# JialeTao/MRFA

Hardware: AMD Instinct MI355X
Metric: frames/sec (256x256 source+driving pair) fwd+bwd (higher is better)
Workload: dtype f32; 1 GPU; vox1.yaml MTIA (TokenPose_B) prior + DenseMotion + RaftFlow refinement, 256x256, bs=8/GPU, fwd+bwd+clip+Adam, train-mode BN, surrogate L1 loss; global_batch=8, parallelism=dp1, prior=mtia, background_predictor=False, sync_bn=False, launch=hipGraph, optimizer=FlatAdam (K20), mfma=bf16x6

## Files before the change

### mrfa_amd/csrc/common.h

```cpp
#pragma once
#include <hip/hip_runtime.h>
#include <stdio.h>
#include <string.h>
#include "mrfa_hip.h"

typedef float f32x16 __attribute__((ext_vector_type(16)));
typedef float f32x4 __attribute__((ext_vector_type(4)));

void mrfa_set_error(const char* fmt, ...);

struct MrfaTuning {
    int conv_small;
    int conv_halo, conv_halo_min_tiles, conv_halo_pr, conv_halo_phase, conv_halo_bn256, conv_halo_bn192, conv_halo_bn64_fill;
    int conv_lean, conv_lean_min_wgs, conv_lean_geo, gemm_lean;
    int wgrad_halo, wgrad_halo_min_wgs, wgrad_halo_target_wgs, wgrad_halo_phase, wgrad_lean;
    int conv_fewout3, attention_mfma;
};
extern MrfaTuning g_tune;

struct HaloGeo { int PR, BN; bool phase; };

enum class ConvFamily { lean, gemm_lean, small, halo, halo_dgrad, rows_split, rows_f32, refused };
struct ConvPlan {
    ConvFamily family;
    char error[256];
    long long M;
    int KT;
    int lean_geo, gemm_cfg, small_tm, small_tn;
    HaloGeo halo;
    int BM, BN, splitk;
    bool w8;
    bool fused;
    bool fin_in_launch;
    bool reads_w;
    int last_config;
    bool groups_ok, bst_ok, stride2_ok, mask_ok, phase_dgrad_ok;
};
ConvPlan plan_conv(const mrfa_conv_params& p);

enum class WgradFamily { lean, small, halo, tiled, refused };
struct WgradPlan {
    WgradFamily family;
    char error[192];
    long long M;
    bool lean, small;
    bool groups_ok, stride2_ok;
};
WgradPlan plan_wgrad(const mrfa_wgrad_params& p);

int mrfa_conv_split_launch(hipStream_t st, const mrfa_conv_params& p, int KT, long long M, int splitk, int BN);
bool mrfa_conv_halo_eligible(const mrfa_conv_params& p, HaloGeo* geo);
int mrfa_conv_halo_launch(hipStream_t st, const mrfa_conv_params& p, const HaloGeo& geo);
int mrfa_wgrad_split_launch(hipStream_t st, const mrfa_wgrad_params& p, dim3 grid, long long M, long long kps, int tiles_n, int nsplit, int inner,
                            int total_splits, int taps, long long partial_stride, int BM, int BN);

bool mrfa_wgrad_halo_eligible(const mrfa_wgrad_params& p);
int mrfa_wgrad_halo_launch(hipStream_t st, const mrfa_wgrad_params& p);

bool mrfa_fewout3_wgrad(hipStream_t st, const float* x, int ldx, int N, int H, int W, int Cin, const float* dy, int lddy, int Cout, int R, int pad,
                        float* dw, float* dbias, int* rc);

int mrfa_conv_lean_pick(const mrfa_conv_params& p);
int mrfa_conv_lean_launch(hipStream_t st, const mrfa_conv_params& p, int geo);
int mrfa_gemm_lean_pick(const mrfa_conv_params& p, long long M);
int mrfa_gemm_lean_launch(hipStream_t st, const mrfa_conv_params& p, long long M, int cfg);

bool mrfa_conv_small_eligible(const mrfa_conv_params& p, long long M);
int mrfa_conv_small_launch(hipStream_t st, const mrfa_conv_params& p, long long M, int tm, int tn);

bool mrfa_attention_mfma_ok(int d, int n, const void* qkv, int ld, const void* out, int ldo, const void* dout, int lddo, const void* dqkv, int lddq);
int mrfa_attention_fwd_mfma(hipStream_t st, const float* qkv, int ld, int B, int n, int heads, int d, float scale, float* out, int ldo, float* lse);
int mrfa_attention_bwd_mfma(hipStream_t st, const float* qkv, int ld, const float* out, int ldo, const float* dout, int lddo, const float* lse,
                            float* delta, int B, int n, int heads, int d, float scale, float* dqkv, int lddq);

bool mrfa_wgrad_lean_eligible(const mrfa_wgrad_params& p);
int mrfa_wgrad_lean_multi(hipStream_t st, const mrfa_wgrad_params* ps, int n, unsigned char* taken);

bool mrfa_wgrad_small_eligible(const mrfa_wgrad_params& p, long long M);
int mrfa_wgrad_small_launch(hipStream_t st, const mrfa_wgrad_params& p, long long M);

#define MRFA_CHECK_ARG(cond, ...)                      \
    do {                                               \
        if (!(cond)) {                                 \
            mrfa_set_error(__VA_ARGS__);               \
            return 1;                                  \
        }                                              \
    } while (0)

#define MRFA_CHECK_LAUNCH(name)                                                   \
    do {                                                                          \
        hipError_t e_ = hipGetLastError();                                        \
        if (e_ != hipSuccess) {                                                   \
            mrfa_set_error("%s: launch failed: %s", name, hipGetErrorString(e_)); \
            return 2;                                                             \
        }                                                                         \
    } while (0)

static inline bool aligned16(const void* p) { return (reinterpret_cast<uintptr_t>(p) & 15u) == 0; }
static inline int cdiv(long long a, long long b) { return (int)((a + b - 1) / b); }
// ... 107 lines not shown
```

### mrfa_amd/csrc/conv_plan.hip

```cpp
#include "common.h"
#include <stdarg.h>

MrfaTuning g_tune = {
     1,
     1,  128,  0,  1,  1,
     1,  1,
     1,  128,  -1,
     1,
     1,  192,  256,  1,
     1,
     1,  1,
};

enum TuneKind { T_ON, T_INT, T_NONNEG, T_NONNEG_ON, T_LEVEL, T_POS };
static const struct { const char* key; int* field; TuneKind kind; } TUNING_KEYS[] = {
    {"conv_small", &g_tune.conv_small, T_ON},
    {"conv_halo", &g_tune.conv_halo, T_ON},
    {"conv_halo_min_tiles", &g_tune.conv_halo_min_tiles, T_INT},
    {"conv_halo_pr", &g_tune.conv_halo_pr, T_INT},
    {"conv_halo_phase", &g_tune.conv_halo_phase, T_ON},
    {"conv_halo_bn256", &g_tune.conv_halo_bn256, T_ON},
    {"conv_halo_bn192", &g_tune.conv_halo_bn192, T_ON},
    {"conv_halo_bn64_fill", &g_tune.conv_halo_bn64_fill, T_ON},
    {"conv_lean", &g_tune.conv_lean, T_ON},
    {"conv_lean_min_wgs", &g_tune.conv_lean_min_wgs, T_NONNEG},
    {"conv_lean_geo", &g_tune.conv_lean_geo, T_INT},
    {"gemm_lean", &g_tune.gemm_lean, T_LEVEL},
    {"wgrad_halo", &g_tune.wgrad_halo, T_ON},
    {"wgrad_halo_min_wgs", &g_tune.wgrad_halo_min_wgs, T_NONNEG},
    {"wgrad_halo_target_wgs", &g_tune.wgrad_halo_target_wgs, T_POS},
    {"wgrad_halo_phase", &g_tune.wgrad_halo_phase, T_NONNEG_ON},
    {"wgrad_lean", &g_tune.wgrad_lean, T_ON},
    {"conv_fewout3", &g_tune.conv_fewout3, T_ON},
    {"attention_mfma", &g_tune.attention_mfma, T_ON},
};

extern "C" int mrfa_set_tuning(const char* key, int value) {
    if (!key) return -1;
    for (const auto& k : TUNING_KEYS) {
        if (strcmp(key, k.key)) continue;
        const int prev = *k.field;
        switch (k.kind) {
            case T_ON: *k.field = value != 0; break;
            case T_INT: *k.field = value; break;
            case T_NONNEG: if (value >= 0) *k.field = value; break;
            case T_NONNEG_ON: if (value >= 0) *k.field = value != 0; break;
            case T_LEVEL: if (value >= 0) *k.field = value > 2 ? 2 : value; break;
            case T_POS: if (value > 0) *k.field = value; break;
        }
        return prev;
    }
    return -1;
}

namespace {
constexpr int BK = 32;

template <typename Plan>
Plan& refuse(Plan& c, const char* fmt, ...) {
    va_list ap;
    va_start(ap, fmt);
    vsnprintf(c.error, sizeof(c.error), fmt, ap);
    va_end(ap);
    c.family = decltype(c.family)::refused;
    return c;
}

void plan_rows(ConvPlan& c, const mrfa_conv_params& p, int mode) {
    const bool flat = p.kflat > 0;
    const long long M = c.M;
    const int KT = c.KT;
    const int nb = p.nbatch > 1 ? p.nbatch : 1;
    int BN = 128;
    {
        const int cands[4] = {128, 96, 64, 32};
        const double pen[4] = {1.0, 1.08, 1.16, 1.3};
        double best = 1e18;
        for (int i = 0; i < 4; ++i) {
            if (cands[i] == 96 && flat) continue;
            const double cost = (double)cdiv(p.Cout, cands[i]) * cands[i] * pen[i];
            if (cost < best) { best = cost; BN = cands[i]; }
        }
    }
    if (mode >= 1 && !flat && p.Cout >= 32) BN = p.Cout <= 64 ? 64 : 128;
    auto ntiles = [&](int bm, int bn) { return ((M + bm - 1) / bm) * cdiv(p.Cout, bn) * nb; };
    int BM = 128;
    if (BN == 96 && ntiles(128, 96) < 384) BN = 128;
    if (BN == 128) { if (M <= 32) BM = 32; else if (M <= 64) BM = 64; }
    else if (BN == 64 && M <= 64) BM = 64;
    int splitk = 1;
    const bool auto_split = (p.splitk == 0);
    if (p.splitk > 1) splitk = p.splitk;
    {
        const bool short_k_big_m = KT < 32 && M > 4096;
        const bool grouped_stats = p.groups > 1 && p.stats && !(p.sk_ticket && !p.accumulate);
        const int max_split = (auto_split && !short_k_big_m && !grouped_stats) ? (KT / 2 > 0 ? KT / 2 : 1) : 1;
        long long t = ntiles(BM, BN);
        if (t < 384 && !(short_k_big_m && t >= 128)) {
            const bool half_target = auto_split && p.sk_ticket && !p.accumulate && KT >= 72 && KT <= 320 && BM == 128 && t >= 8 && t <= 16;
            int want = (int)(((half_target ? 256 : 512) + t - 1) / t);
            if (auto_split) splitk = want <= max_split ? want : max_split;
            const int min_bm = (BN == 128) ? 32 : (BN == 64 ? 64 : 128);
            while (!half_target && ntiles(BM, BN) * splitk < 384 && BM > min_bm) {
                BM >>= 1;
                if (auto_split) {
                    t = ntiles(BM, BN);
                    want = (int)((512 + t - 1) / t);
                    splitk = want <= max_split ? want : max_split;
                }
            }
            if (splitk < 1) splitk = 1;
        }
    }
    bool w8 = false;
    if (p.tile) {
        BM = p.tile >> 16; BN = p.tile & 0x7fff; w8 = (p.tile & 0x8000) != 0;
        if (p.splitk >= 1) splitk = p.splitk;
// ... 134 lines not shown
```

### mrfa_amd/csrc/sample.hip

```cpp
#include "mfma_bf16.h"

namespace {

struct Taps {
    int x0, y0;
    float fx, fy;
};

__device__ __forceinline__ Taps make_taps(float ix, float iy) {
    Taps t;
    const float fx0 = floorf(ix), fy0 = floorf(iy);
    t.x0 = (int)fx0;
    t.y0 = (int)fy0;
    t.fx = ix - fx0;
    t.fy = iy - fy0;
    return t;
}


struct Taps4 {
    size_t o00, o01, o10, o11;
    float w00, w01, w10, w11;
    float fx, fy;
    bool ok00, ok01, ok10, ok11;
// ... 107 lines not shown
        const u32x4 r10 = *reinterpret_cast<const u32x4*>(base + tp.o10 * ldi), r11 = *reinterpret_cast<const u32x4*>(base + tp.o11 * ldi);
        f32x4 a00, b00, a01, b01, a10, b10, a11, b11;
        widen8(r00, a00, b00); widen8(r01, a01, b01); widen8(r10, a10, b10); widen8(r11, a11, b11);
        const f32x4 z = {0.f, 0.f, 0.f, 0.f};
        const f32x4 va = tp.w00 * (tp.ok00 ? a00 : z) + tp.w01 * (tp.ok01 ? a01 : z) + tp.w10 * (tp.ok10 ? a10 : z) + tp.w11 * (tp.ok11 ? a11 : z);
        const f32x4 vb = tp.w00 * (tp.ok00 ? b00 : z) + tp.w01 * (tp.ok01 ? b01 : z) + tp.w10 * (tp.ok10 ? b10 : z) + tp.w11 * (tp.ok11 ? b11 : z);
        float* o = out + (size_t)opix * ldo + c;
        *reinterpret_cast<f32x4*>(o) = va;
        *reinterpret_cast<f32x4*>(o + 4) = vb;
    }
}

template <int LPP>
__global__ __launch_bounds__(256) void grid_sample_bwd_vec_kernel(const float* __restrict__ in, int ldi, long long in_bstride, int in_rep,
                                                                 int Hi, int Wi, int C, const float* __restrict__ grid, int ldg,
                                                                 long long npix, int Ho, int Wo, const float* __restrict__ dout, int lddo,
                                                                 int mode, float* __restrict__ din, int lddi, long long din_bstride,
                                                                 float* __restrict__ dgrid, int lddg) {
    const int chunks = C / (4 * LPP);
    const long long items = npix * chunks;
    const int sub = threadIdx.x % LPP;
    const long long first = (blockIdx.x * (long long)blockDim.x + threadIdx.x) / LPP;
    const long long step = ((long long)gridDim.x * blockDim.x) / LPP;
    const long long iters = (items + step - 1) / step;
    for (long long k = 0; k < iters; ++k) {
        const long long it = first + k * step;
        const bool live = it < items;
        const long long opix = live ? it / chunks : 0;
        const int c = (int)((live ? it : 0) - opix * chunks) * 4 * LPP + sub * 4;
        const int ox = (int)(opix % Wo);
        const long long t = opix / Wo;
        const int oy = (int)(t % Ho);
        const int n = (int)(t / Ho);
        float ix, iy;
        sample_coords(grid, ldg, opix, ox, oy, Wi, Hi, mode, ix, iy);
        float gxs = 0.f, gys = 0.f;
        {
            const Taps4 tp = make_taps4(live ? ix : -2.f, iy, Wi, Hi);
            const f32x4 g = *reinterpret_cast<const f32x4*>(dout + (size_t)opix * lddo + c);
            const size_t ib = (size_t)(n / in_rep) * in_bstride + c;
            const f32x4 z = {0.f, 0.f, 0.f, 0.f};
            const f32x4 l00 = *reinterpret_cast<const f32x4*>(in + ib + tp.o00 * ldi), l01 = *reinterpret_cast<const f32x4*>(in + ib + tp.o01 * ldi);
            const f32x4 l10 = *reinterpret_cast<const f32x4*>(in + ib + tp.o10 * ldi), l11 = *reinterpret_cast<const f32x4*>(in + ib + tp.o11 * ldi);
            const f32x4 v00 = tp.ok00 ? l00 : z, v01 = tp.ok01 ? l01 : z, v10 = tp.ok10 ? l10 : z, v11 = tp.ok11 ? l11 : z;
            if (din) {
                float* db = din + (size_t)(n / in_rep) * din_bstride + c;
#pragma unroll
                for (int q = 0; q < 4; ++q) {
                    if (tp.ok00) atomicAdd(db + tp.o00 * lddi + q, g[q] * tp.w00);
                    if (tp.ok01) atomicAdd(db + tp.o01 * lddi + q, g[q] * tp.w01);
                    if (tp.ok10) atomicAdd(db + tp.o10 * lddi + q, g[q] * tp.w10);
                    if (tp.ok11) atomicAdd(db + tp.o11 * lddi + q, g[q] * tp.w11);
                }
            }
            const bool any = tp.ok00 || tp.ok01 || tp.ok10 || tp.ok11;
#pragma unroll
            for (int q = 0; q < 4; ++q) {
                gxs += g[q] * ((v01[q] - v00[q]) * (1.f - tp.fy) + (v11[q] - v10[q]) * tp.fy);
                gys += g[q] * ((v10[q] - v00[q]) * (1.f - tp.fx) + (v11[q] - v01[q]) * tp.fx);
            }
            if (!any) { gxs = 0.f; gys = 0.f; }
        }
        if (dgrid) {
#pragma unroll
            for (int o = LPP / 2; o > 0; o >>= 1) {
                gxs += __shfl_xor(gxs, o, 64);
                gys += __shfl_xor(gys, o, 64);
            }
            if (sub == 0 && live) {
                const float mx = mode == 0 ? 0.5f * (float)Wi : 1.f, my = mode == 0 ? 0.5f * (float)Hi : 1.f;
                if (chunks == 1) {
                    dgrid[(size_t)opix * lddg] += gxs * mx;
                    dgrid[(size_t)opix * lddg + 1] += gys * my;
                } else {
                    atomicAdd(dgrid + (size_t)opix * lddg, gxs * mx);
                    atomicAdd(dgrid + (size_t)opix * lddg + 1, gys * my);
                }
            }
        }
    }
}

constexpr int GS_RUN = 8;
__global__ __launch_bounds__(256) void grid_sample_bwd_kernel(const float* __restrict__ in, int ldi, long long in_bstride, int in_rep,
                                                             int Hi, int Wi, int C, const float* __restrict__ grid, int ldg,
                                                             long long npix, int Ho, int Wo, const float* __restrict__ dout, int lddo,
                                                             int mode, float* __restrict__ din, int lddi, long long din_bstride,
                                                             float* __restrict__ dgrid, int lddg) {
    const int lane = threadIdx.x & 63;
    const long long wave_id = (blockIdx.x * (long long)blockDim.x + threadIdx.x) >> 6;
    const long long nwaves = ((long long)gridDim.x * blockDim.x) >> 6;
    const int chunks = (C + 63) / 64;
    const int runs_x = (Wo + GS_RUN - 1) / GS_RUN;
    const long long nruns = (long long)(npix / Wo) * runs_x;
    for (long long wi = wave_id; wi < nruns * chunks; wi += nwaves) {
        const long long run = wi / chunks;
        const int c = (int)(wi - run * chunks) * 64 + lane;
        const bool c_ok = c < C;
        const int cc = c_ok ? c : 0;
        const long long rowi = run / runs_x;
        const int ox0 = (int)(run - rowi * runs_x) * GS_RUN;
        const int oy = (int)(rowi % Ho);
        const int n = (int)(rowi / Ho);
        const size_t ib = (size_t)(n / in_rep) * in_bstride + cc;
        float* db = din ? din + (size_t)(n / in_rep) * din_bstride + cc : nullptr;
        float ctop = 0.f, cbot = 0.f;
        long long ptop = -1, pbot = -1;
        const int nrun = min(GS_RUN, Wo - ox0);
        for (int k = 0; k < nrun; ++k) {
            const int ox = ox0 + k;
            const long long opix = rowi * Wo + ox;
            float ix, iy;
            sample_coords(grid, ldg, opix, ox, oy, Wi, Hi, mode, ix, iy);
            const Taps4 tp = make_taps4(ix, iy, Wi, Hi);
            const float g = c_ok ? dout[(size_t)opix * lddo + cc] : 0.f;
            const float l00 = in[ib + tp.o00 * ldi], l01 = in[ib + tp.o01 * ldi], l10 = in[ib + tp.o10 * ldi], l11 = in[ib + tp.o11 * ldi];
            const float v00 = tp.ok00 ? l00 : 0.f, v01 = tp.ok01 ? l01 : 0.f, v10 = tp.ok10 ? l10 : 0.f, v11 = tp.ok11 ? l11 : 0.f;
            if (db) {
                float a00 = g * tp.w00, a10 = g * tp.w10;
                const long long q00 = tp.ok00 ? (long long)tp.o00 : -2, q10 = tp.ok10 ? (long long)tp.o10 : -2;
                if (ptop >= 0) { if (ptop == q00) a00 += ctop; else if (c_ok) atomicAdd(db + ptop * lddi, ctop); }
                if (pbot >= 0) { if (pbot == q10) a10 += cbot; else if (c_ok) atomicAdd(db + pbot * lddi, cbot); }
                if (c_ok) {
                    if (tp.ok00) atomicAdd(db + tp.o00 * lddi, a00);
                    if (tp.ok10) atomicAdd(db + tp.o10 * lddi, a10);
                }
                ptop = tp.ok01 ? (long long)tp.o01 : -1;
                pbot = tp.ok11 ? (long long)tp.o11 : -1;
                ctop = g * tp.w01;
                cbot = g * tp.w11;
            }
            if (dgrid) {
                float gxs = wave_sum(g * ((v01 - v00) * (1.f - tp.fy) + (v11 - v10) * tp.fy));
                float gys = wave_sum(g * ((v10 - v00) * (1.f - tp.fx) + (v11 - v01) * tp.fx));
                if (lane == 0) {
                    const float mx = mode == 0 ? 0.5f * (float)Wi : 1.f, my = mode == 0 ? 0.5f * (float)Hi : 1.f;
                    if (chunks == 1) {
                        dgrid[(size_t)opix * lddg] += gxs * mx;
                        dgrid[(size_t)opix * lddg + 1] += gys * my;
                    } else {
                        atomicAdd(dgrid + (size_t)opix * lddg, gxs * mx);
                        atomicAdd(dgrid + (size_t)opix * lddg + 1, gys * my);
                    }
                }
            }
        }
        if (db && c_ok) {
            if (ptop >= 0) atomicAdd(db + ptop * lddi, ctop);
            if (pbot >= 0) atomicAdd(db + pbot * lddi, cbot);
        }
    }
}

__device__ __forceinline__ void resize_src(int o, int Ni, int No, int& i0, int& i1, float& f) {
    const float s = No > 1 ? (float)(Ni - 1) / (float)(No - 1) : 0.f;
    const float src = s * (float)o;
    i0 = (int)src;
    if (i0 > Ni - 1) i0 = Ni - 1;
    i1 = i0 + (i0 < Ni - 1 ? 1 : 0);
    f = src - (float)i0;
}

__global__ void resize_fwd_kernel(const float* __restrict__ in, int ldi, int N, int Hi, int Wi, int C, float* __restrict__ out, int ldo,
                                  int Ho, int Wo, float mul, int acc, long long total) {
    for (long long i = blockIdx.x * (long long)blockDim.x + threadIdx.x; i < total; i += (long long)gridDim.x * blockDim.x) {
        const long long opix = i / C;
        const int c = (int)(i - opix * C);
        const int ox = (int)(opix % Wo);
        const long long t = opix / Wo;
        const int oy = (int)(t % Ho);
        const long long n = t / Ho;
        int x0, x1, y0, y1;
        float fx, fy;
        resize_src(ox, Wi, Wo, x0, x1, fx);
        resize_src(oy, Hi, Ho, y0, y1, fy);
        const float* b = in + (size_t)n * Hi * Wi * ldi + c;
        const float top = b[((size_t)y0 * Wi + x0) * ldi] * (1.f - fx) + b[((size_t)y0 * Wi + x1) * ldi] * fx;
        const float bot = b[((size_t)y1 * Wi + x0) * ldi] * (1.f - fx) + b[((size_t)y1 * Wi + x1) * ldi] * fx;
        const float v = (top * (1.f - fy) + bot * fy) * mul;
        float* d = out + (size_t)opix * ldo + c;
        *d = acc ? (*d + v) : v;
    }
}

__global__ void resize_bwd_kernel(const float* __restrict__ dout, int lddo, int N, int Hi, int Wi, int C, float* __restrict__ din,
                                  int lddi, int Ho, int Wo, float mul, long long total) {
    for (long long i = blockIdx.x * (long long)blockDim.x + threadIdx.x; i < total; i += (long long)gridDim.x * blockDim.x) {
        const long long opix = i / C;
        const int c = (int)(i - opix * C);
        const int ox = (int)(opix % Wo);
        const long long t = opix / Wo;
        const int oy = (int)(t % Ho);
        const long long n = t / Ho;
        int x0, x1, y0, y1;
        float fx, fy;
        resize_src(ox, Wi, Wo, x0, x1, fx);
        resize_src(oy, Hi, Ho, y0, y1, fy);
        const float g = dout[(size_t)opix * lddo + c] * mul;
        float* b = din + (size_t)n * Hi * Wi * lddi + c;
        atomicAdd(b + ((size_t)y0 * Wi + x0) * lddi, g * (1.f - fx) * (1.f - fy));
        atomicAdd(b + ((size_t)y0 * Wi + x1) * lddi, g * fx * (1.f - fy));
        atomicAdd(b + ((size_t)y1 * Wi + x0) * lddi, g * (1.f - fx) * fy);
        atomicAdd(b + ((size_t)y1 * Wi + x1) * lddi, g * fx * fy);
    }
}

__global__ void resize_bwd_gather_kernel(const float* __restrict__ dout, int lddo, int N, int Hi, int Wi, int C, float* __restrict__ din,
                                         int lddi, int Ho, int Wo, float mul, long long total) {
    const float sy = Ho > 1 ? (float)(Hi - 1) / (float)(Ho - 1) : 0.f, sx = Wo > 1 ? (float)(Wi - 1) / (float)(Wo - 1) : 0.f;
    for (long long i = blockIdx.x * (long long)blockDim.x + threadIdx.x; i < total; i += (long long)gridDim.x * blockDim.x) {
        const long long ipix = i / C;
        const int c = (int)(i - ipix * C);
        const int ix = (int)(ipix % Wi);
        const long long t = ipix / Wi;
        const int iy = (int)(t % Hi);
        const long long n = t / Hi;
        int oy_lo = sy > 0.f ? (int)floorf((float)(iy - 1) / sy) - 1 : 0, oy_hi = sy > 0.f ? (int)ceilf((float)(iy + 1) / sy) + 1 : Ho - 1;
        int ox_lo = sx > 0.f ? (int)floorf((float)(ix - 1) / sx) - 1 : 0, ox_hi = sx > 0.f ? (int)ceilf((float)(ix + 1) / sx) + 1 : Wo - 1;
        oy_lo = max(oy_lo, 0); oy_hi = min(oy_hi, Ho - 1); ox_lo = max(ox_lo, 0); ox_hi = min(ox_hi, Wo - 1);
        const float* g = dout + (size_t)n * Ho * Wo * lddo + c;
        float acc = 0.f;
        for (int oy = oy_lo; oy <= oy_hi; ++oy) {
            int y0, y1; float fy;
            resize_src(oy, Hi, Ho, y0, y1, fy);
            const float wy = (y0 == iy ? 1.f - fy : 0.f) + (y1 == iy ? fy : 0.f);
            if (wy == 0.f) continue;
            float row = 0.f;
            for (int ox = ox_lo; ox <= ox_hi; ++ox) {
                int x0, x1; float fx;
                resize_src(ox, Wi, Wo, x0, x1, fx);
                const float wx = (x0 == ix ? 1.f - fx : 0.f) + (x1 == ix ? fx : 0.f);
                if (wx != 0.f) row += wx * g[((size_t)oy * Wo + ox) * lddo];
            }
            acc += wy * row;
        }
        din[(size_t)ipix * lddi + c] += acc * mul;
    }
}

struct ResizeSumArgs {
    int n;
    int prefix[MRFA_RESIZE_SUM_MAX + 1];
    mrfa_resize_sum_desc d[MRFA_RESIZE_SUM_MAX];
};

template <bool BWD>
__global__ __launch_bounds__(256) void resize_sum_multi_kernel(const ResizeSumArgs a) {
    int lo = 0, hi = a.n;
    while (hi - lo > 1) {
        const int mid = (lo + hi) >> 1;
        if ((int)blockIdx.x >= a.prefix[mid]) lo = mid; else hi = mid;
    }
    const mrfa_resize_sum_desc& d = a.d[lo];
    const long long i = (long long)((int)blockIdx.x - a.prefix[lo]) * 256 + threadIdx.x;
    const long long total = (long long)d.N * d.Hd * d.Wd * d.C;
    if (i >= total) return;
    const long long pix = i / d.C;
    const int c = (int)(i - pix * d.C);
    const int px = (int)(pix % d.Wd);
    const long long t = pix / d.Wd;
    const int py = (int)(t % d.Hd);
    const long long n = t / d.Hd;
    float* dst = d.dst + (size_t)pix * d.ldd + c;
    float v = d.overwrite ? 0.f : *dst;
    bool first = d.overwrite != 0;
    for (int k = 0; k < d.nterm; ++k) {
        const float* __restrict__ src = d.term[k].src;
        const int lds = d.term[k].lds, Hs = d.term[k].Hs, Ws = d.term[k].Ws;
        const float mul = d.term[k].mul;
        float r;
        if (Hs == d.Hd && Ws == d.Wd) {
            r = src[(size_t)pix * lds + c] * mul;
        } else if (!BWD) {
            int x0, x1, y0, y1;
            float fx, fy;
            resize_src(px, Ws, d.Wd, x0, x1, fx);
            resize_src(py, Hs, d.Hd, y0, y1, fy);
            const float* b = src + (size_t)n * Hs * Ws * lds + c;
            const float top = b[((size_t)y0 * Ws + x0) * lds] * (1.f - fx) + b[((size_t)y0 * Ws + x1) * lds] * fx;
            const float bot = b[((size_t)y1 * Ws + x0) * lds] * (1.f - fx) + b[((size_t)y1 * Ws + x1) * lds] * fx;
            r = (top * (1.f - fy) + bot * fy) * mul;
        } else {
            const int Hi = d.Hd, Wi = d.Wd, Ho = Hs, Wo = Ws;
            const float sy = Ho > 1 ? (float)(Hi - 1) / (float)(Ho - 1) : 0.f, sx = Wo > 1 ? (float)(Wi - 1) / (float)(Wo - 1) : 0.f;
            int oy_lo = sy > 0.f ? (int)floorf((float)(py - 1) / sy) - 1 : 0, oy_hi = sy > 0.f ? (int)ceilf((float)(py + 1) / sy) + 1 : Ho - 1;
            int ox_lo = sx > 0.f ? (int)floorf((float)(px - 1) / sx) - 1 : 0, ox_hi = sx > 0.f ? (int)ceilf((float)(px + 1) / sx) + 1 : Wo - 1;
            oy_lo = max(oy_lo, 0); oy_hi = min(oy_hi, Ho - 1); ox_lo = max(ox_lo, 0); ox_hi = min(ox_hi, Wo - 1);
            const float* g = src + (size_t)n * Ho * Wo * lds + c;
            float acc = 0.f;
            for (int oy = oy_lo; oy <= oy_hi; ++oy) {
                int y0, y1; float fy;
                resize_src(oy, Hi, Ho, y0, y1, fy);
                const float wy = (y0 == py ? 1.f - fy : 0.f) + (y1 == py ? fy : 0.f);
                if (wy == 0.f) continue;
                float row = 0.f;
                for (int ox = ox_lo; ox <= ox_hi; ++ox) {
                    int x0, x1; float fx;
                    resize_src(ox, Wi, Wo, x0, x1, fx);
                    const float wx = (x0 == px ? 1.f - fx : 0.f) + (x1 == px ? fx : 0.f);
                    if (wx != 0.f) row += wx * g[((size_t)oy * Wo + ox) * lds];
                }
                acc += wy * row;
            }
            r = acc * mul;
        }
        v = first ? r : v + r;
        first = false;
    }
    *dst = v;
}

template <bool BWD>
__global__ __launch_bounds__(256) void corr_lookup_kernel(const float* __restrict__ vol0, const float* __restrict__ vol1, int Hs, int Ws,
                                                         const float* __restrict__ coords, int ldc, long long Q, int radius,
                                                         float* __restrict__ out, int ldo, const float* __restrict__ dout, int lddo,
                                                         float* __restrict__ dvol0, float* __restrict__ dvol1,
                                                         float* __restrict__ dcoords, int lddc) {
    const int lane = threadIdx.x & 63;
    const long long wave_id = (blockIdx.x * (long long)blockDim.x + threadIdx.x) >> 6;
// ... 148 lines not shown
        const float* pin = in + n * C * (long long)H * W;
        float* pout = out + n * C * (long long)Ho * Wo + (i - n * (long long)Ho * Wo);
        for (int c = 0; c < C; ++c) {
            const float* pc = pin + (long long)c * H * W;
            float v = pc[y0 * W + x0] * wx0 * wy0;
            if (x1ok) v += pc[y0 * W + x1] * wx1 * wy0;
            if (y1ok) v += pc[y1 * W + x0] * wx0 * wy1;
            if (x1ok && y1ok) v += pc[y1 * W + x1] * wx1 * wy1;
            pout[(long long)c * Ho * Wo] = v;
        }
    }
}

}

extern "C" int mrfa_warp_frame_reflect(void* stream, const float* in, int N, int C, int H, int W, const float* grid, int Ho, int Wo, float* out) {
    MRFA_CHECK_ARG(in && grid && out && N > 0 && C > 0 && H > 0 && W > 0 && Ho > 0 && Wo > 0, "warp_frame_reflect: bad args");
    const long long npix = (long long)N * Ho * Wo;
    hipLaunchKernelGGL(warp_frame_reflect_kernel, dim3(stream_grid(npix, 256)), dim3(256), 0, (hipStream_t)stream, in, C, H, W, grid, Ho, Wo, out, npix);
    MRFA_CHECK_LAUNCH("warp_frame_reflect");
    return 0;
}

extern "C" int mrfa_grid_sample_fwd(void* stream, const float* in, int ldi, long long in_bstride, int in_rep, int Hi, int Wi, int C,
                                    const float* grid, int ldg, int N, int Ho, int Wo, float* out, int ldo, int mode) {
    MRFA_CHECK_ARG(in && grid && out && C > 0 && N > 0 && in_rep >= 1 && Hi > 0 && Wi > 0 && Ho > 0 && Wo > 0 && ldi >= C && ldo >= C && ldg >= 2 &&
                   (mode == 0 || mode == 1), "grid_sample_fwd: bad args (sizes must be positive, ldi >= C, ldo >= C, ldg >= 2, mode 0 or 1; C %d, ldi %d, "
                   "ldo %d, ldg %d, mode %d)", C, ldi, ldo, ldg, mode);
    const long long total = (long long)N * Ho * Wo * C;
    const int lpp = C % 256 == 0 ? 64 : (C == 128 ? 32 : (C == 64 ? 16 : 0));
    if (lpp && ldi % 4 == 0 && ldo % 4 == 0 && in_bstride % 4 == 0 && aligned16(in) && aligned16(out)) {
        const long long npix = (long long)N * Ho * Wo;
        dim3 g(stream_grid(total / 4, 256));
#define GSF(L) hipLaunchKernelGGL((grid_sample_fwd_vec_kernel<L>), g, dim3(256), 0, (hipStream_t)stream, in, ldi, in_bstride, in_rep, Hi, Wi, C, \
                                   grid, ldg, npix, Ho, Wo, out, ldo, mode)
        if (lpp == 64) GSF(64); else if (lpp == 32) GSF(32); else GSF(16);
#undef GSF
        MRFA_CHECK_LAUNCH("grid_sample_fwd(vec)");
        return 0;
    }
    hipLaunchKernelGGL(grid_sample_fwd_kernel, dim3(stream_grid(total, 256)), dim3(256), 0, (hipStream_t)stream, in, ldi, in_bstride,
                       in_rep, Hi, Wi, C, grid, ldg, N, Ho, Wo, out, ldo, mode, total);
    MRFA_CHECK_LAUNCH("grid_sample_fwd");
    return 0;
}

extern "C" int mrfa_grid_sample_bf16_fwd(void* stream, const unsigned short* in, int ldi, long long in_bstride, int in_rep, int Hi, int Wi, int C,
                                         const float* grid, int ldg, int N, int Ho, int Wo, float* out, int ldo, int mode) {
    MRFA_CHECK_ARG(in && grid && out && C > 0 && N > 0 && in_rep >= 1 && Hi > 0 && Wi > 0 && Ho > 0 && Wo > 0 && ldi >= C && ldo >= C && ldg >= 2 &&
                   (mode == 0 || mode == 1), "grid_sample_bf16_fwd: bad args");
    MRFA_CHECK_ARG(C % 8 == 0 && ldi % 8 == 0 && in_bstride % 8 == 0 && ldo % 4 == 0 && aligned16(in) && aligned16(out),
                   "grid_sample_bf16_fwd: needs C %% 8 == 0, ldi %% 8 == 0, in_bstride %% 8 == 0, ldo %% 4 == 0 and 16-byte aligned in / out "
                   "(C %d, ldi %d, ldo %d)", C, ldi, ldo);
    const long long npix = (long long)N * Ho * Wo;
    const int c8 = C / 8;
    const int lpp = c8 % 64 == 0 ? 64 : (c8 == 32 ? 32 : (c8 == 16 ? 16 : (c8 == 8 ? 8 : 1)));
    dim3 g(stream_grid(npix * c8, 256));
#define GSH(L) hipLaunchKernelGGL((grid_sample_bf16_fwd_kernel<L>), g, dim3(256), 0, (hipStream_t)stream, in, ldi, in_bstride, in_rep, Hi, Wi, C, \
                                   grid, ldg, npix, Ho, Wo, out, ldo, mode)
    if (lpp == 64) GSH(64); else if (lpp == 32) GSH(32); else if (lpp == 16) GSH(16); else if (lpp == 8) GSH(8); else GSH(1);
#undef GSH
    MRFA_CHECK_LAUNCH("grid_sample_bf16_fwd");
    return 0;
}

extern "C" int mrfa_grid_sample_bwd(void* stream, const float* in, int ldi, long long in_bstride, int in_rep, int Hi, int Wi, int C,
                                    const float* grid, int ldg, int N, int Ho, int Wo, const float* dout, int lddo, int mode,
                                    float* din, int lddi, long long din_bstride, float* dgrid, int lddg) {
    MRFA_CHECK_ARG(in && grid && dout && C > 0 && N > 0 && in_rep >= 1 && Hi > 0 && Wi > 0 && Ho > 0 && Wo > 0 && ldi >= C && lddo >= C && ldg >= 2 &&
                   (!din || lddi >= C) && (!dgrid || lddg >= 2) && (mode == 0 || mode == 1),
                   "grid_sample_bwd: bad args (sizes must be positive, ldi >= C, lddo >= C, ldg >= 2, lddi >= C with din, lddg >= 2 with dgrid, mode 0 or 1; "
                   "C %d, ldi %d, lddo %d, ldg %d, lddi %d, lddg %d, mode %d)", C, ldi, lddo, ldg, lddi, lddg, mode);
    const long long npix = (long long)N * Ho * Wo;
    const int lpp = C % 256 == 0 ? 64 : (C == 128 ? 32 : (C == 64 ? 16 : 0));
    if (lpp && !din && ldi % 4 == 0 && lddo % 4 == 0 && in_bstride % 4 == 0 && aligned16(in) && aligned16(dout)) {
        dim3 g(stream_grid(npix * C / 4, 256));
#define GSB(L) hipLaunchKernelGGL((grid_sample_bwd_vec_kernel<L>), g, dim3(256), 0, (hipStream_t)stream, in, ldi, in_bstride, in_rep, Hi, Wi, C, \
                                   grid, ldg, npix, Ho, Wo, dout, lddo, mode, din, lddi, din_bstride, dgrid, lddg)
        if (lpp == 64) GSB(64); else if (lpp == 32) GSB(32); else GSB(16);
#undef GSB
        MRFA_CHECK_LAUNCH("grid_sample_bwd(vec)");
        return 0;
    }
    const long long waves = (long long)N * Ho * cdiv(Wo, GS_RUN) * cdiv(C, 64);
    hipLaunchKernelGGL(grid_sample_bwd_kernel, dim3(stream_grid(waves * 64, 256)), dim3(256), 0, (hipStream_t)stream, in, ldi, in_bstride,
                       in_rep, Hi, Wi, C, grid, ldg, npix, Ho, Wo, dout, lddo, mode, din, lddi, din_bstride, dgrid, lddg);
    MRFA_CHECK_LAUNCH("grid_sample_bwd");
    return 0;
}

extern "C" int mrfa_resize_bilinear_fwd(void* stream, const float* in, int ldi, int N, int Hi, int Wi, int C, float* out, int ldo,
                                        int Ho, int Wo, float scale_mul, int accumulate) {
    MRFA_CHECK_ARG(in && out && C > 0 && N > 0 && Hi > 0 && Wi > 0 && Ho > 0 && Wo > 0 && ldi >= C && ldo >= C,
                   "resize_fwd: bad args (sizes must be positive, ldi >= C, ldo >= C; C %d, ldi %d, ldo %d, %d x %d -> %d x %d)", C, ldi, ldo, Hi, Wi, Ho, Wo);
    const long long total = (long long)N * Ho * Wo * C;
    hipLaunchKernelGGL(resize_fwd_kernel, dim3(stream_grid(total, 256)), dim3(256), 0, (hipStream_t)stream, in, ldi, N, Hi, Wi, C, out, ldo,
                       Ho, Wo, scale_mul, accumulate, total);
    MRFA_CHECK_LAUNCH("resize_fwd");
    return 0;
}

extern "C" int mrfa_resize_bilinear_bwd(void* stream, const float* dout, int lddo, int N, int Hi, int Wi, int C, float* din, int lddi,
                                        int Ho, int Wo, float scale_mul) {
    MRFA_CHECK_ARG(dout && din && C > 0 && N > 0 && Hi > 0 && Wi > 0 && Ho > 0 && Wo > 0 && lddo >= C && lddi >= C,
                   "resize_bwd: bad args (sizes must be positive, lddo >= C, lddi >= C; C %d, lddo %d, lddi %d, %d x %d -> %d x %d)", C, lddo, lddi, Hi, Wi, Ho, Wo);
    if (Ho >= Hi && Wo >= Wi) {
        const long long total_in = (long long)N * Hi * Wi * C;
        hipLaunchKernelGGL(resize_bwd_gather_kernel, dim3(stream_grid(total_in, 256)), dim3(256), 0, (hipStream_t)stream, dout, lddo, N, Hi,
                           Wi, C, din, lddi, Ho, Wo, scale_mul, total_in);
        MRFA_CHECK_LAUNCH("resize_bwd_gather");
        return 0;
    }
    const long long total = (long long)N * Ho * Wo * C;
    hipLaunchKernelGGL(resize_bwd_kernel, dim3(stream_grid(total, 256)), dim3(256), 0, (hipStream_t)stream, dout, lddo, N, Hi, Wi, C, din,
                       lddi, Ho, Wo, scale_mul, total);
    MRFA_CHECK_LAUNCH("resize_bwd");
    return 0;
}

static int resize_sum_launch(void* stream, const mrfa_resize_sum_desc* descs, int n, bool bwd, const char* what) {
    MRFA_CHECK_ARG(n >= 0 && (n == 0 || descs), "%s: bad args", what);
    for (int base = 0; base < n; base += MRFA_RESIZE_SUM_MAX) {
        ResizeSumArgs a;
        a.n = n - base < MRFA_RESIZE_SUM_MAX ? n - base : MRFA_RESIZE_SUM_MAX;
        int blocks = 0;
        for (int i = 0; i < a.n; ++i) {
            const mrfa_resize_sum_desc& d = descs[base + i];
            MRFA_CHECK_ARG(d.dst && d.N > 0 && d.Hd > 0 && d.Wd > 0 && d.C > 0 && d.nterm >= 1 && d.nterm <= MRFA_RESIZE_SUM_TERMS, "%s: record %d: bad sizes / term count", what, base + i);
            for (int k = 0; k < d.nterm; ++k) {
                MRFA_CHECK_ARG(d.term[k].src && d.term[k].Hs > 0 && d.term[k].Ws > 0, "%s: record %d term %d: null source / bad size", what, base + i, k);
                if (bwd) MRFA_CHECK_ARG(d.term[k].Hs >= d.Hd && d.term[k].Ws >= d.Wd, "%s: record %d term %d: the backward takes up-sampling (or same-size) terms only", what, base + i, k);
            }
            a.d[i] = d;
            a.prefix[i] = blocks;
            const long long total = (long long)d.N * d.Hd * d.Wd * d.C;
            MRFA_CHECK_ARG(total < (1ll << 31) - 256 && blocks + (total + 255) / 256 < (1ll << 30), "%s: record %d too large", what, base + i);
            blocks += (int)((total + 255) / 256);
        }
        a.prefix[a.n] = blocks;
        if (bwd) hipLaunchKernelGGL((resize_sum_multi_kernel<true>), dim3(blocks), dim3(256), 0, (hipStream_t)stream, a);
        else hipLaunchKernelGGL((resize_sum_multi_kernel<false>), dim3(blocks), dim3(256), 0, (hipStream_t)stream, a);
        MRFA_CHECK_LAUNCH(what);
    }
    return 0;
}

extern "C" int mrfa_resize_sum_multi(void* stream, const mrfa_resize_sum_desc* descs, int n) {
    return resize_sum_launch(stream, descs, n, false, "resize_sum_multi");
}

extern "C" int mrfa_resize_sum_multi_bwd(void* stream, const mrfa_resize_sum_desc* descs, int n) {
    return resize_sum_launch(stream, descs, n, true, "resize_sum_multi_bwd");
}

extern "C" int mrfa_corr_lookup_fwd(void* stream, const float* vol0, const float* vol1, int Hs, int Ws, const float* coords, int ldc,
                                    long long Q, int radius, float* out, int ldo) {
    MRFA_CHECK_ARG(radius >= 0 && radius <= 3, "corr_lookup: window must fit one wave (0 <= radius <= 3, got %d)", radius);
    MRFA_CHECK_ARG(vol0 && vol1 && coords && out && Q > 0 && Hs >= 2 && Ws >= 2 && ldc >= 2 && ldo >= 2 * (2 * radius + 1) * (2 * radius + 1),
                   "corr_lookup_fwd: bad args (Hs, Ws >= 2, ldc >= 2, ldo >= 2 (2r+1)^2; Hs %d, Ws %d, ldc %d, ldo %d, radius %d)", Hs, Ws, ldc, ldo, radius);
    hipLaunchKernelGGL((corr_lookup_kernel<false>), dim3(stream_grid(Q * 64, 256)), dim3(256), 0, (hipStream_t)stream, vol0, vol1, Hs, Ws,
                       coords, ldc, Q, radius, out, ldo, nullptr, 0, nullptr, nullptr, nullptr, 0);
    MRFA_CHECK_LAUNCH("corr_lookup_fwd");
    return 0;
}

static int corr_direct_launch(void* stream, const float* q, int ldq, const float* k0, int ldk0, const float* k1, int ldk1, int N, int k_rep, int h1, int w1,
                              int Hs, int Ws, int D, const float* coords, int ldc, int radius, float scale, float* out, int ldo) {
    MRFA_CHECK_ARG(radius >= 0 && radius <= 3, "corr_direct: the window's lattice must fit one wave (0 <= radius <= 3, got %d)", radius);
    MRFA_CHECK_ARG(q && k0 && k1 && coords && out && N > 0 && h1 > 0 && w1 > 0 && D > 0, "corr_direct_fwd: bad args (null pointer or non-positive size; "
                   "N %d, h1 %d, w1 %d, D %d)", N, h1, w1, D);
    MRFA_CHECK_ARG(Hs >= 2 && Ws >= 2 && Hs % 2 == 0 && Ws % 2 == 0, "corr_direct_fwd: Hs and Ws must be even and >= 2 (the pooled level is Hs/2 x Ws/2; "
                   "Hs %d, Ws %d)", Hs, Ws);
    MRFA_CHECK_ARG(ldc >= 2 && ldo >= 2 * (2 * radius + 1) * (2 * radius + 1) && ldq >= D && ldk0 >= D && ldk1 >= D,
                   "corr_direct_fwd: a leading dimension is below its channel count (ldc >= 2, ldo >= 2 (2r+1)^2, ldq / ldk0 / ldk1 >= D; ldc %d, ldo %d, "
                   "ldq %d, ldk0 %d, ldk1 %d, D %d, radius %d)", ldc, ldo, ldq, ldk0, ldk1, D, radius);
    MRFA_CHECK_ARG(D % 4 == 0 && ldq % 4 == 0 && ldk0 % 4 == 0 && ldk1 % 4 == 0 && aligned16(q) && aligned16(k0) && aligned16(k1),
                   "corr_direct_fwd: needs D %% 4 == 0, ldq / ldk0 / ldk1 %% 4 == 0 and 16-byte aligned q / k0 / k1 (16-byte loads; D %d, ldq %d, ldk0 %d, "
                   "ldk1 %d)", D, ldq, ldk0, ldk1);
    const long long QI = (long long)h1 * w1, Q = (long long)N * QI, QK = QI * k_rep;
    long long blocks = ((Q + 3) / 4 + 7) / 8 * 8;
    if (blocks > 2048) blocks = 2048;
    const long long per = (Q + blocks * 4 - 1) / (blocks * 4);
#define CDK(S) hipLaunchKernelGGL((corr_direct_kernel<S>), dim3((unsigned)blocks), dim3(256), 0, (hipStream_t)stream, q, ldq, k0, ldk0, k1, ldk1, Q, QK, \
                                  Hs, Ws, D, coords, ldc, radius, scale, per, out, ldo)
    if (D == 256) CDK(8); else CDK(0);
#undef CDK
    MRFA_CHECK_LAUNCH("corr_direct_fwd");
    return 0;
// ... 28 lines not shown
```

Before: 103.9 pairs/s.

## Multi-row grid_sample backward and vectorized bilinear resize kernels

The scalar grid_sample backward now handles R output rows per wave, merging atomic adds across vertically adjacent rows. It can also loop over all channel chunks in one wave so the dgrid reduction is written once rather than atomically per chunk, with R and chunk grouping picked by a wave-count heuristic. Separately, new float4-vectorized kernels cover bilinear resize forward and gather-style backward. These aim to cut atomic traffic, scalar loads and launch-level overhead, at the cost of more registers and fewer waves.

```diff
diff --git a/mrfa_amd/csrc/common.h b/mrfa_amd/csrc/common.h
--- a/mrfa_amd/csrc/common.h
+++ b/mrfa_amd/csrc/common.h
@@ -15,6 +15,7 @@
     int conv_lean, conv_lean_min_wgs, conv_lean_geo, gemm_lean;
     int wgrad_halo, wgrad_halo_min_wgs, wgrad_halo_target_wgs, wgrad_halo_phase, wgrad_lean;
     int conv_fewout3, attention_mfma;
+    int gs_bwd_rows;
 };
 extern MrfaTuning g_tune;
 
diff --git a/mrfa_amd/csrc/conv_plan.hip b/mrfa_amd/csrc/conv_plan.hip
--- a/mrfa_amd/csrc/conv_plan.hip
+++ b/mrfa_amd/csrc/conv_plan.hip
@@ -10,6 +10,7 @@
      1,  192,  256,  1,
      1,
      1,  1,
+     0,
 };
 
 enum TuneKind { T_ON, T_INT, T_NONNEG, T_NONNEG_ON, T_LEVEL, T_POS };
@@ -33,6 +34,7 @@
     {"wgrad_lean", &g_tune.wgrad_lean, T_ON},
     {"conv_fewout3", &g_tune.conv_fewout3, T_ON},
     {"attention_mfma", &g_tune.attention_mfma, T_ON},
+    {"gs_bwd_rows", &g_tune.gs_bwd_rows, T_INT},
 };
 
 extern "C" int mrfa_set_tuning(const char* key, int value) {
diff --git a/mrfa_amd/csrc/sample.hip b/mrfa_amd/csrc/sample.hip
--- a/mrfa_amd/csrc/sample.hip
+++ b/mrfa_amd/csrc/sample.hip
@@ -213,72 +213,121 @@
 }
 
 constexpr int GS_RUN = 8;
+constexpr int GS_BWD_MIN_WAVES = 4096;
+
+__device__ __forceinline__ float wave_uniform(float v) { return __int_as_float(__builtin_amdgcn_readfirstlane(__float_as_int(v))); }
+
+template <int R>
 __global__ __launch_bounds__(256) void grid_sample_bwd_kernel(const float* __restrict__ in, int ldi, long long in_bstride, int in_rep,
                                                              int Hi, int Wi, int C, const float* __restrict__ grid, int ldg,
                                                              long long npix, int Ho, int Wo, const float* __restrict__ dout, int lddo,
                                                              int mode, float* __restrict__ din, int lddi, long long din_bstride,
-                                                             float* __restrict__ dgrid, int lddg) {
+                                                             float* __restrict__ dgrid, int lddg, int cpw) {
     const int lane = threadIdx.x & 63;
     const long long wave_id = (blockIdx.x * (long long)blockDim.x + threadIdx.x) >> 6;
     const long long nwaves = ((long long)gridDim.x * blockDim.x) >> 6;
     const int chunks = (C + 63) / 64;
+    const int groups = (chunks + cpw - 1) / cpw;
     const int runs_x = (Wo + GS_RUN - 1) / GS_RUN;
-    const long long nruns = (long long)(npix / Wo) * runs_x;
-    for (long long wi = wave_id; wi < nruns * chunks; wi += nwaves) {
-        const long long run = wi / chunks;
-        const int c = (int)(wi - run * chunks) * 64 + lane;
-        const bool c_ok = c < C;
-        const int cc = c_ok ? c : 0;
-        const long long rowi = run / runs_x;
-        const int ox0 = (int)(run - rowi * runs_x) * GS_RUN;
-        const int oy = (int)(rowi % Ho);
-        const int n = (int)(rowi / Ho);
-        const size_t ib = (size_t)(n / in_rep) * in_bstride + cc;
-        float* db = din ? din + (size_t)(n / in_rep) * din_bstride + cc : nullptr;
-        float ctop = 0.f, cbot = 0.f;
-        long long ptop = -1, pbot = -1;
+    const int strips_y = (Ho + R - 1) / R;
+    const long long nruns = (npix / Wo / Ho) * strips_y * runs_x;
+    for (long long wi = wave_id; wi < nruns * groups; wi += nwaves) {
+        const long long run = wi / groups;
+        const int ch0 = (int)(wi - run * groups) * cpw;
+        const int nch = min(cpw, chunks - ch0);
+        const long long strip = run / runs_x;
+        const int ox0 = (int)(run - strip * runs_x) * GS_RUN;
+        const int oy0 = (int)(strip % strips_y) * R;
+        const int n = (int)(strip / strips_y);
         const int nrun = min(GS_RUN, Wo - ox0);
-        for (int k = 0; k < nrun; ++k) {
-            const int ox = ox0 + k;
-            const long long opix = rowi * Wo + ox;
-            float ix, iy;
-            sample_coords(grid, ldg, opix, ox, oy, Wi, Hi, mode, ix, iy);
-            const Taps4 tp = make_taps4(ix, iy, Wi, Hi);
-            const float g = c_ok ? dout[(size_t)opix * lddo + cc] : 0.f;
-            const float l00 = in[ib + tp.o00 * ldi], l01 = in[ib + tp.o01 * ldi], l10 = in[ib + tp.o10 * ldi], l11 = in[ib + tp.o11 * ldi];
-            const float v00 = tp.ok00 ? l00 : 0.f, v01 = tp.ok01 ? l01 : 0.f, v10 = tp.ok10 ? l10 : 0.f, v11 = tp.ok11 ? l11 : 0.f;
-            if (db) {
-                float a00 = g * tp.w00, a10 = g * tp.w10;
-                const long long q00 = tp.ok00 ? (long long)tp.o00 : -2, q10 = tp.ok10 ? (long long)tp.o10 : -2;
-                if (ptop >= 0) { if (ptop == q00) a00 += ctop; else if (c_ok) atomicAdd(db + ptop * lddi, ctop); }
-                if (pbot >= 0) { if (pbot == q10) a10 += cbot; else if (c_ok) atomicAdd(db + pbot * lddi, cbot); }
-                if (c_ok) {
-                    if (tp.ok00) atomicAdd(db + tp.o00 * lddi, a00);
-                    if (tp.ok10) atomicAdd(db + tp.o10 * lddi, a10);
+        float gxa = 0.f, gya = 0.f;
+        for (int ch = 0; ch < nch; ++ch) {
+            const int c = (ch0 + ch) * 64 + lane;
+            const bool c_ok = c < C;
+            const int cc = c_ok ? c : 0;
+            const size_t ib = (size_t)(n / in_rep) * in_bstride + cc;
+            float* db = din ? din + (size_t)(n / in_rep) * din_bstride + cc : nullptr;
+            float ctop[R], cbot[R];
+            long long ptop[R], pbot[R];
+#pragma unroll
+            for (int r = 0; r < R; ++r) { ctop[r] = 0.f; cbot[r] = 0.f; ptop[r] = -1; pbot[r] = -1; }
+            for (int k = 0; k < nrun; ++k) {
+                const int ox = ox0 + k;
+                Taps4 tp[R];
+                float g[R], l00[R], l01[R], l10[R], l11[R];
+#pragma unroll
+                for (int r = 0; r < R; ++r) {
+                    const bool row_ok = oy0 + r < Ho;
+                    const int oy = row_ok ? oy0 + r : Ho - 1;
+                    const long long opix = ((long long)n * Ho + oy) * Wo + ox;
+                    float ix, iy;
+                    sample_coords(grid, ldg, opix, ox, oy, Wi, Hi, mode, ix, iy);
+                    ix = wave_uniform(ix); iy = wave_uniform(iy);
+                    tp[r] = make_taps4(row_ok ? ix : -2.f, iy, Wi, Hi);
+                    g[r] = c_ok ? dout[(size_t)opix * lddo + cc] : 0.f;
+                    l00[r] = in[ib + tp[r].o00 * ldi]; l01[r] = in[ib + tp[r].o01 * ldi];
+                    l10[r] = in[ib + tp[r].o10 * ldi]; l11[r] = in[ib + tp[r].o11 * ldi];
                 }
-                ptop = tp.ok01 ? (long long)tp.o01 : -1;
-                pbot = tp.ok11 ? (long long)tp.o11 : -1;
-                ctop = g * tp.w01;
-                cbot = g * tp.w11;
-            }
-            if (dgrid) {
-                float gxs = wave_sum(g * ((v01 - v00) * (1.f - tp.fy) + (v11 - v10) * tp.fy));
-                float gys = wave_sum(g * ((v10 - v00) * (1.f - tp.fx) + (v11 - v01) * tp.fx));
-                if (lane == 0) {
-                    const float mx = mode == 0 ? 0.5f * (float)Wi : 1.f, my = mode == 0 ? 0.5f * (float)Hi : 1.f;
-                    if (chunks == 1) {
-                        dgrid[(size_t)opix * lddg] += gxs * mx;
-                        dgrid[(size_t)opix * lddg + 1] += gys * my;
-                    } else {
-                        atomicAdd(dgrid + (size_t)opix * lddg, gxs * mx);
-                        atomicAdd(dgrid + (size_t)opix * lddg + 1, gys * my);
+                if (db) {
+                    float a00[R], a10[R];
+                    long long q00[R], q10[R];
+#pragma unroll
+                    for (int r = 0; r < R; ++r) {
+                        a00[r] = g[r] * tp[r].w00; a10[r] = g[r] * tp[r].w10;
+                        q00[r] = tp[r].ok00 ? (long long)tp[r].o00 : -2; q10[r] = tp[r].ok10 ? (long long)tp[r].o10 : -2;
+                        if (ptop[r] >= 0) { if (ptop[r] == q00[r]) a00[r] += ctop[r]; else if (c_ok) atomicAdd(db + ptop[r] * lddi, ctop[r]); }
+                        if (pbot[r] >= 0) { if (pbot[r] == q10[r]) a10[r] += cbot[r]; else if (c_ok) atomicAdd(db + pbot[r] * lddi, cbot[r]); }
+                    }
+#pragma unroll
+                    for (int r = 0; r < R; ++r) {
+                        if (r > 0 && q10[r - 1] >= 0 && q10[r - 1] == q00[r]) a00[r] += a10[r - 1];
+                        const bool down = r + 1 < R && q10[r] >= 0 && q10[r] == q00[r + 1 < R ? r + 1 : r];
+                        if (c_ok) {
+                            if (tp[r].ok00) atomicAdd(db + tp[r].o00 * lddi, a00[r]);
+                            if (tp[r].ok10 && !down) atomicAdd(db + tp[r].o10 * lddi, a10[r]);
+                        }
+                        ptop[r] = tp[r].ok01 ? (long long)tp[r].o01 : -1;
+                        pbot[r] = tp[r].ok11 ? (long long)tp[r].o11 : -1;
+                        ctop[r] = g[r] * tp[r].w01;
+                        cbot[r] = g[r] * tp[r].w11;
                     }
                 }
-            }
-        }
-        if (db && c_ok) {
-            if (ptop >= 0) atomicAdd(db + ptop * lddi, ctop);
-            if (pbot >= 0) atomicAdd(db + pbot * lddi, cbot);
+                if (dgrid) {
+#pragma unroll
+                    for (int r = 0; r < R; ++r) {
+                        const float v00 = tp[r].ok00 ? l00[r] : 0.f, v01 = tp[r].ok01 ? l01[r] : 0.f;
+                        const float v10 = tp[r].ok10 ? l10[r] : 0.f, v11 = tp[r].ok11 ? l11[r] : 0.f;
+                        const float gxs = wave_sum(g[r] * ((v01 - v00) * (1.f - tp[r].fy) + (v11 - v10) * tp[r].fy));
+                        const float gys = wave_sum(g[r] * ((v10 - v00) * (1.f - tp[r].fx) + (v11 - v01) * tp[r].fx));
+                        if (lane == k * R + r) { gxa += gxs; gya += gys; }
+                    }
+                }
+            }
+            if (db) {
+#pragma unroll
+                for (int r = 0; r < R; ++r) {
+                    if (r > 0 && pbot[r - 1] >= 0 && pbot[r - 1] == ptop[r]) ctop[r] += cbot[r - 1];
+                    const bool down = r + 1 < R && pbot[r] >= 0 && pbot[r] == ptop[r + 1 < R ? r + 1 : r];
+                    if (c_ok) {
+                        if (ptop[r] >= 0) atomicAdd(db + ptop[r] * lddi, ctop[r]);
+                        if (pbot[r] >= 0 && !down) atomicAdd(db + pbot[r] * lddi, cbot[r]);
+                    }
+                }
+            }
+        }
+        if (dgrid) {
+            const int k = lane / R, r = lane % R;
+            if (k < nrun && oy0 + r < Ho) {
+                const size_t opix = (size_t)(((long long)n * Ho + oy0 + r) * Wo + ox0 + k);
+                const float mx = mode == 0 ? 0.5f * (float)Wi : 1.f, my = mode == 0 ? 0.5f * (float)Hi : 1.f;
+                if (groups == 1) {
+                    dgrid[opix * lddg] += gxa * mx;
+                    dgrid[opix * lddg + 1] += gya * my;
+                } else {
+                    atomicAdd(dgrid + opix * lddg, gxa * mx);
+                    atomicAdd(dgrid + opix * lddg + 1, gya * my);
+                }
+            }
         }
     }
 }
@@ -366,6 +415,98 @@
             acc += wy * row;
         }
         din[(size_t)ipix * lddi + c] += acc * mul;
+    }
+}
+
+typedef float f32x4u __attribute__((ext_vector_type(4), aligned(4)));
+__device__ __forceinline__ f32x4 load4u(const float* p) { return *reinterpret_cast<const f32x4u*>(p); }
+__device__ __forceinline__ float pick(const f32x4 v, int i) { return i == 0 ? v.x : (i == 1 ? v.y : (i == 2 ? v.z : v.w)); }
+
+__global__ __launch_bounds__(256) void resize_fwd_vec_kernel(const float* __restrict__ in, int ldi, int N, int Hi, int Wi, int C, float* __restrict__ out,
+                                                            int ldo, int Ho, int Wo, float mul, int acc, long long items) {
+    const int quads = (C + 3) / 4;
+    for (long long i = blockIdx.x * (long long)blockDim.x + threadIdx.x; i < items; i += (long long)gridDim.x * blockDim.x) {
+        const long long opix = i / quads;
+        const int c = (int)(i - opix * quads) * 4;
+        const int nq = C - c;
+        const int cb = nq >= 4 ? c : C - 4;
+        const int ox = (int)(opix % Wo);
+        const long long t = opix / Wo;
+        const int oy = (int)(t % Ho);
+        const long long n = t / Ho;
+        int x0, x1, y0, y1;
+        float fx, fy;
+        resize_src(ox, Wi, Wo, x0, x1, fx);
+        resize_src(oy, Hi, Ho, y0, y1, fy);
+        const float* b = in + (size_t)n * Hi * Wi * ldi + cb;
+        const f32x4 v00 = load4u(b + ((size_t)y0 * Wi + x0) * ldi), v01 = load4u(b + ((size_t)y0 * Wi + x1) * ldi);
+        const f32x4 v10 = load4u(b + ((size_t)y1 * Wi + x0) * ldi), v11 = load4u(b + ((size_t)y1 * Wi + x1) * ldi);
+        const f32x4 top = v00 * (1.f - fx) + v01 * fx;
+        const f32x4 bot = v10 * (1.f - fx) + v11 * fx;
+        const f32x4 v = (top * (1.f - fy) + bot * fy) * mul;
+        float* d = out + (size_t)opix * ldo + c;
+        if (nq >= 4) {
+            *reinterpret_cast<f32x4*>(d) = acc ? *reinterpret_cast<const f32x4*>(d) + v : v;
+        } else {
+            for (int q = 0; q < nq; ++q) d[q] = acc ? d[q] + pick(v, q + c - cb) : pick(v, q + c - cb);
+        }
+    }
+}
+
+constexpr int RS_CAND = 12;
+template <int NC>
+__global__ __launch_bounds__(256) void resize_bwd_gather_vec_kernel(const float* __restrict__ dout, int lddo, int N, int Hi, int Wi, int C,
+                                                                   float* __restrict__ din, int lddi, int Ho, int Wo, float mul, long long items) {
+    const float sy = Ho > 1 ? (float)(Hi - 1) / (float)(Ho - 1) : 0.f, sx = Wo > 1 ? (float)(Wi - 1) / (float)(Wo - 1) : 0.f;
+    const int quads = (C + 3) / 4;
+    for (long long i = blockIdx.x * (long long)blockDim.x + threadIdx.x; i < items; i += (long long)gridDim.x * blockDim.x) {
+        const long long ipix = i / quads;
+        const int c = (int)(i - ipix * quads) * 4;
+        const int nq = C - c;
+        const int cb = nq >= 4 ? c : C - 4;
+        const int ix = (int)(ipix % Wi);
+        const long long t = ipix / Wi;
+        const int iy = (int)(t % Hi);
+        const long long n = t / Hi;
+        int oy_lo = sy > 0.f ? (int)floorf((float)(iy - 1) / sy) - 1 : 0, oy_hi = sy > 0.f ? (int)ceilf((float)(iy + 1) / sy) + 1 : Ho - 1;
+        int ox_lo = sx > 0.f ? (int)floorf((float)(ix - 1) / sx) - 1 : 0, ox_hi = sx > 0.f ? (int)ceilf((float)(ix + 1) / sx) + 1 : Wo - 1;
+        oy_lo = max(oy_lo, 0); oy_hi = min(oy_hi, Ho - 1); ox_lo = max(ox_lo, 0); ox_hi = min(ox_hi, Wo - 1);
+        float wx[NC];
+        for (;; ++ox_lo) {
+            int x0, x1; float fx;
+            resize_src(ox_lo, Wi, Wo, x0, x1, fx);
+            wx[0] = (x0 == ix ? 1.f - fx : 0.f) + (x1 == ix ? fx : 0.f);
+            if (wx[0] != 0.f || ox_lo >= ox_hi) break;
+        }
+#pragma unroll
+        for (int j = 1; j < NC; ++j) {
+            int x0, x1; float fx;
+            resize_src(min(ox_lo + j, Wo - 1), Wi, Wo, x0, x1, fx);
+            wx[j] = ox_lo + j <= ox_hi ? (x0 == ix ? 1.f - fx : 0.f) + (x1 == ix ? fx : 0.f) : 0.f;
+        }
+        const float* g = dout + (size_t)n * Ho * Wo * lddo + cb;
+        const f32x4 z = {0.f, 0.f, 0.f, 0.f};
+        f32x4 acc = z;
+        for (int oy = oy_lo; oy <= oy_hi; ++oy) {
+            int y0, y1; float fy;
+            resize_src(oy, Hi, Ho, y0, y1, fy);
+            const float wy = (y0 == iy ? 1.f - fy : 0.f) + (y1 == iy ? fy : 0.f);
+            if (wy == 0.f) continue;
+            f32x4 v[NC];
+#pragma unroll
+            for (int j = 0; j < NC; ++j) v[j] = load4u(g + ((size_t)oy * Wo + min(ox_lo + j, Wo - 1)) * lddo);
+            f32x4 row = z;
+#pragma unroll
+            for (int j = 0; j < NC; ++j) row += wx[j] * (wx[j] != 0.f ? v[j] : z);
+            acc += wy * row;
+        }
+        acc = acc * mul;
+        float* d = din + (size_t)ipix * lddi + c;
+        if (nq >= 4) {
+            *reinterpret_cast<f32x4*>(d) = *reinterpret_cast<const f32x4*>(d) + acc;
+        } else {
+            for (int q = 0; q < nq; ++q) d[q] += pick(acc, q + c - cb);
+        }
     }
 }
 
@@ -680,17 +821,36 @@
         MRFA_CHECK_LAUNCH("grid_sample_bwd(vec)");
         return 0;
     }
-    const long long waves = (long long)N * Ho * cdiv(Wo, GS_RUN) * cdiv(C, 64);
-    hipLaunchKernelGGL(grid_sample_bwd_kernel, dim3(stream_grid(waves * 64, 256)), dim3(256), 0, (hipStream_t)stream, in, ldi, in_bstride,
-                       in_rep, Hi, Wi, C, grid, ldg, npix, Ho, Wo, dout, lddo, mode, din, lddi, din_bstride, dgrid, lddg);
+    const int chunks = cdiv(C, 64);
+    const auto waves_of = [&](int r, int cpw) { return (long long)N * cdiv(Ho, r) * cdiv(Wo, GS_RUN) * cdiv(chunks, cpw); };
+    int R = g_tune.gs_bwd_rows;
+    if (R != 1 && R != 2 && R != 4) R = waves_of(2, 1) >= GS_BWD_MIN_WAVES ? 2 : 1;
+    const int cpw = waves_of(R, chunks) >= GS_BWD_MIN_WAVES ? chunks : 1;
+    dim3 g(stream_grid(waves_of(R, cpw) * 64, 256));
+#define GSS(RR) hipLaunchKernelGGL((grid_sample_bwd_kernel<RR>), g, dim3(256), 0, (hipStream_t)stream, in, ldi, in_bstride, in_rep, Hi, Wi, C, \
+                                   grid, ldg, npix, Ho, Wo, dout, lddo, mode, din, lddi, din_bstride, dgrid, lddg, cpw)
+    if (R == 4) GSS(4); else if (R == 2) GSS(2); else GSS(1);
+#undef GSS
     MRFA_CHECK_LAUNCH("grid_sample_bwd");
     return 0;
 }
+
+static bool resize_vec_ok(int C, const void* a, int lda, const void* b, int ldb) {
+    return C >= 4 && lda % 4 == 0 && ldb % 4 == 0 && aligned16(a) && aligned16(b);
+}
+static int resize_candidates(int Ni, int No) { return Ni == 1 ? No : cdiv(2LL * (No - 1), Ni - 1) + 1; }
 
 extern "C" int mrfa_resize_bilinear_fwd(void* stream, const float* in, int ldi, int N, int Hi, int Wi, int C, float* out, int ldo,
                                         int Ho, int Wo, float scale_mul, int accumulate) {
     MRFA_CHECK_ARG(in && out && C > 0 && N > 0 && Hi > 0 && Wi > 0 && Ho > 0 && Wo > 0 && ldi >= C && ldo >= C,
                    "resize_fwd: bad args (sizes must be positive, ldi >= C, ldo >= C; C %d, ldi %d, ldo %d, %d x %d -> %d x %d)", C, ldi, ldo, Hi, Wi, Ho, Wo);
+    if (resize_vec_ok(C, in, ldi, out, ldo)) {
+        const long long items = (long long)N * Ho * Wo * cdiv(C, 4);
+        hipLaunchKernelGGL(resize_fwd_vec_kernel, dim3(stream_grid(items, 256)), dim3(256), 0, (hipStream_t)stream, in, ldi, N, Hi, Wi, C, out, ldo,
+                           Ho, Wo, scale_mul, accumulate, items);
+        MRFA_CHECK_LAUNCH("resize_fwd(vec)");
+        return 0;
+    }
     const long long total = (long long)N * Ho * Wo * C;
     hipLaunchKernelGGL(resize_fwd_kernel, dim3(stream_grid(total, 256)), dim3(256), 0, (hipStream_t)stream, in, ldi, N, Hi, Wi, C, out, ldo,
                        Ho, Wo, scale_mul, accumulate, total);
@@ -702,6 +862,16 @@
                                         int Ho, int Wo, float scale_mul) {
     MRFA_CHECK_ARG(dout && din && C > 0 && N > 0 && Hi > 0 && Wi > 0 && Ho > 0 && Wo > 0 && lddo >= C && lddi >= C,
                    "resize_bwd: bad args (sizes must be positive, lddo >= C, lddi >= C; C %d, lddo %d, lddi %d, %d x %d -> %d x %d)", C, lddo, lddi, Hi, Wi, Ho, Wo);
+    if (Ho >= Hi && Wo >= Wi && resize_vec_ok(C, dout, lddo, din, lddi) && resize_candidates(Wi, Wo) <= RS_CAND && resize_candidates(Hi, Ho) <= RS_CAND) {
+        const long long items = (long long)N * Hi * Wi * cdiv(C, 4);
+        const int nc = resize_candidates(Wi, Wo);
+#define RSG(NC) hipLaunchKernelGGL((resize_bwd_gather_vec_kernel<NC>), dim3(stream_grid(items, 256)), dim3(256), 0, (hipStream_t)stream, dout, lddo, N, Hi, \
+                                   Wi, C, din, lddi, Ho, Wo, scale_mul, items)
+        if (nc <= 6) RSG(6); else if (nc <= 10) RSG(10); else RSG(12);
+#undef RSG
+        MRFA_CHECK_LAUNCH("resize_bwd_gather(vec)");
+        return 0;
+    }
     if (Ho >= Hi && Wo >= Wi) {
         const long long total_in = (long long)N * Hi * Wi * C;
         hipLaunchKernelGGL(resize_bwd_gather_kernel, dim3(stream_grid(total_in, 256)), dim3(256), 0, (hipStream_t)stream, dout, lddo, N, Hi,
```

After: 103.5 pairs/s. No clear change (-0.4%).
